# mkeeter/fidget

Hardware: AMD Instinct MI355X
Metric: Mvoxel/s (interval+point eval) on prospero.vm 1024^3 (higher is better)
Workload: dtype f32; 1 GPU; prospero.vm 3D heightmap+normals 1024^3, HipShape render hints (the library's tiles: 128/32/8, or 32/8 when the root level has few tiles), world_to_model=I

## Files before the change

fidget_amd/csrc/capi_core.hpp:

```cpp
struct DevBuf {
    void* p = nullptr;
    size_t cap = 0;
    hipError_t ensure(size_t bytes) {
        if (bytes <= cap) return hipSuccess;
        if (p) (void)hipFree(p);
        p = nullptr; cap = 0;
        hipError_t e = hipMalloc(&p, bytes);
        if (e == hipSuccess) cap = bytes;
        return e;
    }
    void release() { if (p) (void)hipFree(p); p = nullptr; cap = 0; }
};

static std::atomic<uint64_t> g_tape_serial{1};
struct BoundCache {
    struct Entry {
        uint64_t hash = 0, used = 0;
        std::vector<uint64_t> key;
        std::shared_ptr<const fhip_tape> tape;
    };
    std::mutex lock;
    std::vector<Entry> entries;
    uint64_t clock = 0;
};
// ... 52 lines not shown
#define X(name, dflt) {#name, &FhOptions::name},
    FH_OPTION_LIST(X)
#undef X
};
static void options_from_env(FhOptions& o) {
    for (const FhOptionEntry& e : FH_OPTION_TABLE) {
        std::string var = "FHIP_";
        for (const char* c = e.name; *c; c++) var += (char)toupper((unsigned char)*c);
        if (const char* v = getenv(var.c_str())) o.*(e.field) = *v ? atoi(v) : 1;
    }
}

struct FrameBufs {
    DevBuf state, arena, leaves, leaf_table, zbuf, normals, fp_lists, mind, squeue, slots[2], leaves_b, leaf_table_b, fp_lists_b, chw[2], tvals, topch, chwr, gscratch, rare_scratch;
    DevBuf queue[FH_MAX_LEVELS];
    uint32_t frame_stamp = 0;
    uint64_t resident_serial = 0;
    uint32_t resident_groups = 0;
    uint32_t forked = 0;
    bool async_pending = false;
    hipEvent_t ev_done = nullptr;
    bool ev_done_valid = false;
    std::shared_ptr<const fhip_tape> bound_hold;
    void release_all() {
        DevBuf* bufs[] = {&state, &arena, &leaves, &leaf_table, &zbuf, &normals, &fp_lists, &mind, &squeue, &slots[0], &slots[1],
                          &leaves_b, &leaf_table_b, &fp_lists_b, &chw[0], &chw[1], &tvals, &topch, &chwr, &gscratch, &rare_scratch};
        for (DevBuf* b : bufs) b->release();
        for (auto& q : queue) q.release();
        if (ev_done) (void)hipEventDestroy(ev_done);
        ev_done = nullptr;
        bound_hold.reset();
    }
};
struct fhip_ctx : FrameBufs {
    FhOptions opt;
#define FH_EXTRA_SETS 4
    FrameBufs others[FH_EXTRA_SETS];
    uint32_t extra_sets = 3;
    bool frame_pipeline = true;
    hipStream_t stream_pre = nullptr;
    uint32_t pre_turn = 0;
    hipEvent_t ev_rest_fork = nullptr, ev_rest_join = nullptr;
    hipEvent_t ev_pre = nullptr, ev_l0 = nullptr, ev_l1 = nullptr;
    hipModule_t asm_mod = nullptr;
    hipFunction_t asm_fn[FH_ASM_COUNT] = {};
    bool use_asm = true;
    bool probe = false;
// ... 204 lines not shown
```

fidget_amd/csrc/capi_render.hpp:

```cpp
static fhip_status bind_inputs(fhip_ctx* ctx, const fhip_tape* tape, const int32_t* axis_slots, const uint64_t* keys,
                               const float* vals, uint32_t n, FhRender& P) {
    const fh::HostTape& t = tape->t;
    std::vector<char> bound(FH_MAX_INPUTS, 0);
    for (uint32_t s = 0; s < FH_MAX_INPUTS; s++) { P.in_kind[s] = 3; P.in_value[s] = 0.0f; }
    for (int a = 0; a < 3; a++) {
        const int s = axis_slots ? axis_slots[a] : t.vars.axis[a];
        if (s >= 0 && s < FH_MAX_INPUTS) { P.in_kind[s] = (uint32_t)a; bound[s] = 1; }
    }
    for (uint32_t i = 0; i < n; i++) {
        const int s = axis_slots ? (int)keys[i] : t.vars.slot_of(3, keys[i]);
        if (s >= 0 && s < FH_MAX_INPUTS) { P.in_value[s] = vals[i]; bound[s] = 1; }
    }
    for (uint32_t s = 0; s < t.n_vars; s++)
        if (!bound[s]) return fail(ctx, FHIP_ERR_MISSING_VAR, "a variable of the shape has no value");
    return FHIP_OK;
}

struct HostSpans {
    double t[8] = {0, 0, 0, 0, 0, 0, 0, 0};
    uint64_t n = 0;
    std::chrono::steady_clock::time_point last;
    void start() { last = std::chrono::steady_clock::now(); }
    void mark(int k) { const auto now = std::chrono::steady_clock::now(); t[k] += std::chrono::duration<double, std::micro>(now - last).count(); last = now; }
    void frame() {
// ... 309 lines not shown
        kp.big = 1; kp.max_choices = R.S.P.max_choices;
        (void)launch_asm(ctx, fs.on(), FH_ASM_PRUNE1, bound, &kp, sizeof(kp));
    }
}
static void tiles_hip(fhip_ctx* ctx, const RenderSetup& R, FhRenderState* dS, int level, hipStream_t st) {
    const int gs = blocks_for(ctx, R.lds_tiles_small, 8), gb = blocks_big(ctx, R, R.lds_tiles_big, 8);
    if (level > 0 && R.full) FH_KLAUNCH((k_teval3d<true, false>), dim3(gs), dim3(WAVE), R.lds_tiles_small, st, dS, level);
    else if (level > 0) FH_KLAUNCH((k_teval3d<false, false>), dim3(gs), dim3(WAVE), R.lds_tiles_small, st, dS, level);
    if (R.full) FH_KLAUNCH((k_teval3d<true, true>), dim3(gb), dim3(WAVE), R.lds_tiles_big, st, dS, level);
    else FH_KLAUNCH((k_teval3d<false, true>), dim3(gb), dim3(WAVE), R.lds_tiles_big, st, dS, level);
}
static void launch_tiles_mono(fhip_ctx* ctx, const RenderSetup& R, FhRenderState* dS, int level, bool is3d, hipStream_t st) {
    const int gs = blocks_for(ctx, R.lds_tiles_small, 8), gb = blocks_big(ctx, R, R.lds_tiles_big, 8);
    launch(ctx, st, FHIP_K_TILES, [&] {
        if (is3d) { if (R.full) FH_LAUNCH_TILES(true, true, true, gb, R.lds_tiles_big); else FH_LAUNCH_TILES(true, false, true, gb, R.lds_tiles_big); }
        else { if (R.full) FH_LAUNCH_TILES(false, true, true, gb, R.lds_tiles_big); else FH_LAUNCH_TILES(false, false, true, gb, R.lds_tiles_big); }
    });
    if (level > 0)
        launch(ctx, st, FHIP_K_TILES, [&] {
            if (is3d) { if (R.full) FH_LAUNCH_TILES(true, true, false, gs, R.lds_tiles_small); else FH_LAUNCH_TILES(true, false, false, gs, R.lds_tiles_small); }
            else { if (R.full) FH_LAUNCH_TILES(false, true, false, gs, R.lds_tiles_small); else FH_LAUNCH_TILES(false, false, false, gs, R.lds_tiles_small); }
        });
}
static void launch_tiles(fhip_ctx* ctx, const RenderSetup& R, const LevelPlan& L, FhRenderState* dS, int level, bool is3d, FrameStreams& fs) {
    if (L.path == LevelPlan::MONO) return launch_tiles_mono(ctx, R, dS, level, is3d, fs.on());
    const int gp = ctx->n_cu * 8;
    launch(ctx, fs.on(), FHIP_K_TILES, [&] {
        if (is3d) FH_KLAUNCH(k_tsetup3d, dim3(gp), dim3(WAVE), 0, fs.on(), dS, level);
        else FH_KLAUNCH(k_tsetup2d, dim3(gp), dim3(WAVE), 0, fs.on(), dS, level);
    });
    launch(ctx, fs.on(), FHIP_K_TILES, [&] {
        if (L.path == LevelPlan::GROUPS) tiles_by_groups(ctx, R, dS, fs.on());
        else if (L.path == LevelPlan::ASM) tiles_asm(ctx, R, L, dS, level, fs);
        else tiles_hip(ctx, R, dS, level, fs.on());
    });
    const bool last = level + 1 == (int)R.S.P.n_levels;
    const int gpush = last ? ctx->n_cu * L.push_mul : gp;
    launch(ctx, fs.on(), FHIP_K_TILES, [&] {
        const uint32_t rb = L.rare ? FH_RARE_BLOCKS : 0u;
        if (is3d) FH_KLAUNCH(k_tpush3d, dim3(gpush + rb, last ? 1 : 17), dim3(WAVE), 0, fs.on(), dS, level, rb, rare_file(ctx, dS, L.rare_stride), L.rare_stride);
        else {
            if (!R.classify_only) FH_KLAUNCH(k_tpush2d, dim3(gpush), dim3(WAVE), 0, fs.on(), dS, level);
            const uint32_t slots_max = R.S.qcap[level] * ((level == 0 && R.groups) ? R.S.n_tgroups : 1u);
            FH_KLAUNCH(k_tfill2d, dim3(64, slots_max), dim3(256), 0, fs.on(), dS, level);
        }
    });
}

static fhip_status render2d_frame(fhip_ctx* ctx, const fhip_tape* tape, const fhip_render2d_config* cfg, float* out,
                                  int out_is_device) {
    if (ctx->is_cancelled()) return fail(ctx, FHIP_ERR_CANCELLED, "cancelled");
// ... 88 lines not shown
    HIP_TRY(ctx, hipEventRecord(ctx->ev_done, ctx->stream));
    ctx->ev_done_valid = true;
    if (!out_is_device) {
        HIP_TRY(ctx, hipMemcpyAsync(out, d_out, npix * 4, hipMemcpyDeviceToHost, ctx->stream));
        return finish_render(ctx);
    }
    return FHIP_OK;
}

static void slab_begin(fhip_ctx* ctx, const RenderSetup& R, const FrameSchedule& F, FhRenderState* dS, int k, hipStream_t st) {
    const FhRender& P = R.S.P;
    const uint32_t pre = R.S.pre_levels, n_groups = R.groups_per_slab, n32 = ((P.width + 31) / 32) * ((P.height + 31) / 32);
    launch(ctx, st, FHIP_K_OTHER, [&] {
        const bool pyr3 = P.n_levels == 3 && P.tiles[2] == 8 && P.tiles[1] == 32 && P.tiles[0] == 128 && n32 <= 1024;
        const bool rebuild = k != F.slab_first;
        const bool pyr2 = P.n_levels == 2 && P.tiles[1] == 8 && P.tiles[0] == 32 && pre == 1;
        if (rebuild && pyr2) { FH_KLAUNCH(k_slab_begin2, dim3(n32 + F.reset_blocks), dim3(256), 0, st, dS, n32, F.table_words, (uint32_t)k, n_groups); return; }
        if (rebuild && pyr3 && pre == 2) { FH_KLAUNCH(k_slab_begin3, dim3(n32 + F.reset_blocks), dim3(256), 0, st, dS, n32, F.table_words, (uint32_t)k, n_groups); return; }
        FH_KLAUNCH(k_reset_slab, dim3(F.reset_blocks * 4), dim3(WAVE), 0, st, dS, F.table_words, (uint32_t)k, n_groups, (pyr3 && rebuild) ? 1u : 0u);
        if (rebuild && pyr3) FH_KLAUNCH(k_minpyramid3, dim3(n32), dim3(256), 0, st, dS);
        else if (rebuild) FH_KLAUNCH(k_minpyramid, dim3(P.roots_x * P.roots_y), dim3(256), 0, st, dS);
    });
}
static fhip_status tile_step(fhip_ctx* ctx, const RenderSetup& R, const FrameSchedule& F, FrameStreams& fs, FhRenderState* dS, int k, int idx) {
    fs.cur = F.tiles;
    if (F.pipe && idx >= (int)F.NC) HIP_TRY(ctx, hipStreamWaitEvent(fs.on(), ctx->ev_leaves[idx - (int)F.NC], 0));
    slab_begin(ctx, R, F, dS, k, fs.on());
    for (uint32_t l = R.S.pre_levels; l < R.S.P.n_levels; l++) launch_tiles(ctx, R, F.level[l], dS, (int)l, true, fs);
    if (F.pipe) HIP_TRY(ctx, hipEventRecord(ctx->ev_tiles[idx], fs.on()));
    fs.cur = CALLER;
    return FHIP_OK;
}
static void classify_work(fhip_ctx* ctx, const RenderSetup& R, const FrameSchedule& F, FhRenderState* dS, hipStream_t st) {
    const uint32_t class_blocks = (R.n_footprints + FH_CLASSIFY_FP - 1) / FH_CLASSIFY_FP;
    if (F.by_list && F.rare && R.S.P.max_regs > R.S.leaf_asm_regs)
        launch(ctx, st, FHIP_K_OTHER, [&] { FH_KLAUNCH(k_classify3d, dim3(FH_RARE_BLOCKS), dim3(WAVE), 0, st, dS, 1, 0u, rare_file(ctx, dS, F.rare_stride), F.rare_stride); });
    else if (!F.by_list) launch(ctx, st, FHIP_K_OTHER, [&] {
        FH_KLAUNCH(k_classify3d, dim3(class_blocks + (F.rare ? FH_RARE_BLOCKS : 0u)), dim3(R.S.P.slab / 8 > 16 ? 256 : WAVE), 0, st, dS, R.asm_points ? 1 : 0, class_blocks,
                   rare_file(ctx, dS, F.rare_stride), F.rare_stride);
    });
    if (R.S.P.max_regs > R.S.leaf_asm_regs && !F.rare)
        launch(ctx, st, FHIP_K_POINTS, [&] {
            const int g = blocks_big(ctx, R, R.lds_points_big, 16);
            if (R.full) FH_KLAUNCH((k_leaves3d<2, 0, 1, true>), dim3(g), dim3(WAVE), R.lds_points_big, st, dS);
            else FH_KLAUNCH((k_leaves3d<2, 0, 1, false>), dim3(g), dim3(WAVE), R.lds_points_big, st, dS);
        });
}
static void leaf_work(fhip_ctx* ctx, const RenderSetup& R, const FrameSchedule& F, FhRenderState* dS, uint32_t sk, hipStream_t st) {
    launch(ctx, st, FHIP_K_POINTS, [&] {
        if (F.leaf_walk == FrameSchedule::HIP_LEAVES) {
            const int per_cu = R.full ? 8 : 16;
// ... 24 lines not shown
    launch(ctx, st, FHIP_K_NORMALS, [&] {
        const int gs = blocks_for(ctx, R.lds_normals_small, 8), gb = blocks_big(ctx, R, R.lds_normals_big, 8);
        const int which = R.asm_points_t ? FH_ASM_NORMALS_T : FH_ASM_NORMALS;
        if (F.by_list) {
            if (F.rare && R.S.P.max_regs > R.S.norm_asm_regs)
                FH_KLAUNCH(k_hits3d, dim3(FH_RARE_BLOCKS), dim3(WAVE), 0, st, dS, z_lo, z_hi, R.hit_bucket_cap, 0u, rare_file(ctx, dS, F.rare_stride), F.rare_stride);
            KaNormals kn = {dS, F.list_waves, R.col_slots, z_lo, z_hi, R.hit_bucket_cap, 1u};
            (void)launch_asm(ctx, st, which, kn.n_waves, &kn, sizeof(kn));
        }
        else if (R.asm_normals) {
            const uint32_t hb = std::min<uint32_t>(R.n_footprints, (uint32_t)ctx->n_cu * 64);
            FH_KLAUNCH(k_hits3d, dim3(hb + (F.rare ? FH_RARE_BLOCKS : 0u)), dim3(WAVE), 0, st, dS, z_lo, z_hi, R.hit_bucket_cap, hb, rare_file(ctx, dS, F.rare_stride), F.rare_stride);
            KaNormals kn = {dS, std::max<uint32_t>((uint32_t)(ctx->n_cu * 8) / FH_HIT_BUCKETS, 1u) * FH_HIT_BUCKETS, R.col_slots, z_lo, z_hi, R.hit_bucket_cap, 0};
            (void)launch_asm(ctx, st, which, kn.n_waves, &kn, sizeof(kn));
        }
        else if (R.full) FH_KLAUNCH((k_normals3d<true, false>), dim3(gs), dim3(WAVE), R.lds_normals_small, st, dS, z_lo, z_hi);
        else FH_KLAUNCH((k_normals3d<false, false>), dim3(gs), dim3(WAVE), R.lds_normals_small, st, dS, z_lo, z_hi);
        if (R.S.P.max_regs > R.S.norm_asm_regs && !(F.rare && R.asm_normals)) {
            if (R.full) FH_KLAUNCH((k_normals3d<true, true>), dim3(gb), dim3(WAVE), R.lds_normals_big, st, dS, z_lo, z_hi);
            else FH_KLAUNCH((k_normals3d<false, true>), dim3(gb), dim3(WAVE), R.lds_normals_big, st, dS, z_lo, z_hi);
        }
    });
}
static fhip_status coarse_levels(fhip_ctx* ctx, const RenderSetup& R, const FrameSchedule& F, FrameStreams& fs, FhRenderState* dS) {
    const uint32_t pre = R.S.pre_levels;
    FhFork fork{};
    fork.n = F.NC; fork.mark = F.coarse ? 1u : 0u;
    fork.leaves = (FhLeaf*)ctx->leaves_b.p; fork.leaf_table = (FhLeafRef*)ctx->leaf_table_b.p; fork.fp_lists = (uint32_t*)ctx->fp_lists_b.p;
    fork.leaf_cap = (size_t)R.S.leaf_cap; fork.n_footprints = (size_t)R.n_footprints; fork.hit_words = R.hit_words;
    const bool forked_here = F.coarse && R.zrep;
    if (F.coarse) {
        launch_tiles(ctx, R, F.level[0], dS, 0, true, fs);
        if (pre > 1) {
            HIP_TRY(ctx, hop(fs, F.l1_flags, ctx->ev_l0));
            if (R.zrep) launch(ctx, fs.on(), FHIP_K_OTHER, [&] { FH_KLAUNCH(k_tape_flags, dim3(ctx->n_cu * 4), dim3(WAVE), 0, fs.on(), dS, 1, R.col_depmask, 0, FhFork{}); });
            HIP_TRY(ctx, hop(fs, F.l1, ctx->ev_l0));
            launch_tiles(ctx, R, F.level[1], dS, 1, true, fs);
        }
        HIP_TRY(ctx, hop(fs, F.fork_on, pre > 1 ? ctx->ev_l1 : ctx->ev_l0));
        if (R.zrep) launch(ctx, fs.on(), FHIP_K_OTHER, [&] { FH_KLAUNCH(k_tape_flags, dim3(ctx->n_cu * 8 + 1), dim3(WAVE), 0, fs.on(), dS, (int)pre, R.col_depmask, 1, fork); });
        if (!F.pipe && !forked_here) launch(ctx, fs.on(), FHIP_K_OTHER, [&] { FH_KLAUNCH(k_mark_frame, dim3(1), dim3(1), 0, fs.on(), dS); });
    }
    if (F.pipe) {
        if (!forked_here) FH_KLAUNCH(k_fork_state, dim3(1), dim3(1), 0, fs.on(), dS, fork);
        HIP_TRY(ctx, hipEventRecord(ctx->ev_fork, fs.on()));
        if (F.fork_to_side) HIP_TRY(ctx, hipStreamWaitEvent(fs.s[SIDE], ctx->ev_fork, 0));
    }
    if (F.ev_pre) HIP_TRY(ctx, hop(fs, CALLER, ctx->ev_pre));
    fs.cur = CALLER;
    if (F.fork_to_tail) HIP_TRY(ctx, hipStreamWaitEvent(fs.s[TAIL], ctx->ev_fork, 0));
    return FHIP_OK;
}
static fhip_status render_slabs(fhip_ctx* ctx, const RenderSetup& R, const FrameSchedule& F, FrameStreams& fs, FhRenderState* dS0) {
    auto slab_state = [&](int idx) { return dS0 + (F.pipe ? (uint32_t)idx % F.NC : 0u); };
    for (int idx = 0; F.tiles_first && idx < F.n_rendered; idx++) { const fhip_status st = tile_step(ctx, R, F, fs, slab_state(idx), F.slab_first - idx, idx); if (st) return st; }
    for (int idx = 0; idx < F.n_rendered; idx++) {
        if (ctx->is_cancelled()) return fail(ctx, FHIP_ERR_CANCELLED, "cancelled");
        const int k = F.slab_first - idx;
        FhRenderState* const dS = slab_state(idx);
        if (!F.tiles_first) { const fhip_status st = tile_step(ctx, R, F, fs, dS, k, idx); if (st) return st; }
        if (F.pipe) HIP_TRY(ctx, hipStreamWaitEvent(fs.s[F.leaf], ctx->ev_tiles[idx], 0));
        if (F.aux_edge) HIP_TRY(ctx, hipStreamWaitEvent(fs.s[F.lists], ctx->ev_tiles[idx], 0));
        classify_work(ctx, R, F, dS, fs.s[F.lists]);
        leaf_work(ctx, R, F, dS, (uint32_t)(dS - dS0), fs.s[F.leaf]);
        if (F.aux_edge) { HIP_TRY(ctx, hipEventRecord(ctx->ev_aux[idx], fs.s[F.leaf])); HIP_TRY(ctx, hipStreamWaitEvent(fs.s[F.normals], ctx->ev_aux[idx], 0)); }
        if (F.normals_on) normals_work(ctx, R, F, dS, k, fs.s[F.normals]);
        if (F.pipe) HIP_TRY(ctx, hipEventRecord(ctx->ev_leaves[idx], fs.s[F.normals]));
    }
    if (F.aux_edge && F.n_rendered > 0) HIP_TRY(ctx, hipStreamWaitEvent(fs.s[CALLER], ctx->ev_leaves[F.n_rendered - 1], 0));
    return FHIP_OK;
}

static fhip_status render3d_frame(fhip_ctx* ctx, const fhip_tape* tape, const fhip_render3d_config* cfg, void* out,
                                  int out_is_device, const PartSpec& part) {
    if (ctx->is_cancelled()) return fail(ctx, FHIP_ERR_CANCELLED, "cancelled");
    if (ctx->opt.stats & 2) g_spans.start();
    (void)hipSetDevice(ctx->device);
    RenderSetup R;
    memset(&R.S, 0, sizeof(R.S));
    FhRender& P = R.S.P;
    P.width = cfg->width; P.height = cfg->height; P.depth = cfg->depth; P.z = 0; P.pixel_perfect = 0;
    fhip_status st = bind_inputs(ctx, tape, cfg->axis_slots, cfg->var_keys, cfg->var_values, cfg->n_vars, P);
    if (st) return st;
    const uint32_t size[3] = {cfg->width, cfg->height, cfg->depth};
    float s2w[16];
    const float ident[16] = {1, 0, 0, 0, 0, 1, 0, 0, 0, 0, 1, 0, 0, 0, 0, 1};
    fhip_screen_to_world(size, 3, s2w);
    mat_product(cfg->world_to_model ? cfg->world_to_model : ident, s2w, 4, P.mat);
    const TapeFacts facts = tape_facts(tape);
    const PlanInputs pin = plan_inputs(ctx);
    column_facts(P, facts, pin, R);
    const TileChoice tiles = choose_tiles_3d(cfg->tile_sizes, cfg->n_tile_sizes, size, part.n_shards * part.nx * part.ny, part.nz, R.column_inv, pin.root32_max, pin.no_zrep,
                                             linked_root_tape(facts, pin));
    if (!tiles.valid) return fail(ctx, FHIP_ERR_UNSUPPORTED, "bad tile size list");
    if (tiles.substituted) ctx->substituted_tiles++;
    ScheduleInputs in = schedule_inputs(ctx, out_is_device);
    in.huge = (size_t)std::max<uint32_t>(tape->t.n_regs, 1) * WAVE * 16 > FH_LDS_MAX || tiles_lds(std::max<uint32_t>(tape->t.n_regs, 1), tape->t.n_choices, 64) > FH_LDS_MAX;
    in.whole = part.n_shards == 1 && part.nx * part.ny * part.nz == 1;
    if (frame_pipelined(in)) {
        for (uint32_t i = 0; i < ctx->extra_sets; i++) std::swap(static_cast<FrameBufs&>(*ctx), ctx->others[i]);
        in.frames_queued = ctx->extra_sets > 0 && ctx->others[0].ev_done_valid && hipEventQuery(ctx->others[0].ev_done) == hipErrorNotReady;
        (void)hipGetLastError();
    }
    FH_SPAN(0);
    st = prepare(ctx, tape, facts, true, tiles.ts, part, R);
    if (st) return st;
    FH_SPAN(1);
    in.pre_turn = ctx->pre_turn;
    if (ctx->host_flags) { in.rare_seen = ctx->host_flags[2]; in.last_leaves = ctx->host_flags[3]; }
    const FrameSchedule F = schedule_frame(R, in);
    if (F.takes_turn) ctx->pre_turn++;
    if (F.rare) { HIP_TRY(ctx, ctx->rare_scratch.ensure((size_t)F.rare_stride * FH_RARE_BLOCKS * 4)); ctx->rare_frames++; }
    R.S.leaf_list = F.by_list ? 1u : 0u; ctx->forked = F.pipe ? F.NC : 0;
    FrameStreams fs = frame_streams(ctx, F.root);
    if (F.fpipe && ctx->ev_done_valid) HIP_TRY(ctx, hipStreamWaitEvent(fs.on(), ctx->ev_done, 0));
    const size_t npix = (size_t)cfg->width * cfg->height;
    FhGeometryPixel* d_out = (FhGeometryPixel*)out;
    if (!out_is_device) { HIP_TRY(ctx, ctx->tmp_out.ensure(npix * sizeof(FhGeometryPixel))); d_out = (FhGeometryPixel*)ctx->tmp_out.p; }
    FhRenderState* const dS0 = (FhRenderState*)ctx->state.p;
    const FrameClear clear3[3] = {{ctx->zbuf.p, npix * 8, 0u}, {ctx->normals.p, npix * 12, 0u}, {ctx->mind.p, R.mind_words * 4, 0u}};
    st = upload_frame(ctx, fs.on(), tape, R, clear3);
    if (st) return st;
    FH_SPAN(2);
    st = coarse_levels(ctx, R, F, fs, dS0);
    if (st) return st;
    FH_SPAN(3);
    st = render_slabs(ctx, R, F, fs, dS0);
    if (st) return st;
    FH_SPAN(4);
    launch(ctx, ctx->stream, FHIP_K_OTHER, [&] { FH_KLAUNCH(k_finish3d, dim3(ctx->n_cu * 16), dim3(WAVE), 0, ctx->stream, dS0, d_out, std::max<uint32_t>(ctx->forked, 1u), (uint32_t*)ctx->sticky.p, ctx->host_flags); });
    HIP_TRY(ctx, hipGetLastError());
    if (ctx->launch_failed) { ctx->launch_failed = false; return FHIP_ERR_HIP; }
    ctx->async_pending = out_is_device != 0;
    HIP_TRY(ctx, hipEventRecord(ctx->ev_done, ctx->stream));
    ctx->ev_done_valid = true;
    if (ctx->opt.stats & 2) { g_spans.mark(5); g_spans.frame(); }
    if (!out_is_device) {
        HIP_TRY(ctx, hipMemcpyAsync(out, d_out, npix * sizeof(FhGeometryPixel), hipMemcpyDeviceToHost, ctx->stream));
        return finish_render(ctx);
    }
    return FHIP_OK;
}
static bool lanes_possible(fhip_ctx* ctx, int out_is_device) {
    if (ctx->opt.frame_lanes < 2 || ctx->is_lane || !out_is_device || ctx->profiling || ctx->probe || (ctx->opt.stats & 1)) return false;
    if (!ctx->ev_last_valid) return false;
    const hipError_t q = hipEventQuery(ctx->ev_last);
    (void)hipGetLastError();
    return q == hipErrorNotReady;
}
static void lane_tune_release(fhip_ctx* ctx);
static void lanes_release(fhip_ctx* ctx, bool keep_measurements) {
    if (!keep_measurements) lane_tune_release(ctx);
    for (fhip_ctx* L : ctx->lanes) {
        hipStream_t const s = L->lane_stream_owned ? L->stream : nullptr;
        if (L->lane_done) (void)hipEventDestroy(L->lane_done);
        if (L->lane_copied) (void)hipEventDestroy(L->lane_copied);
        L->lane_img.release();
        fhip_ctx_destroy(L);
// ... 211 lines not shown
```

fidget_amd/csrc/frame_plan.hpp:

```cpp
#pragma once
#include <stddef.h>
#include <stdint.h>
#include <string.h>

#include <algorithm>
#include <vector>

#include "render_state.h"

static const uint32_t VM_TILES_2D[] = {128, 32, 8};
static const uint32_t VM_TILES_3D[] = {128, 64, 32, 16, 8};
static const uint32_t FH_LEAF_REGS = 40, FH_LEAF_REGS_T = 44;
static const uint32_t FH_NORMAL_REGS = 40;
static const uint32_t HIP_TILES_2D[] = {128, 16};
static const uint32_t MID_REGS = 64, MID_CHOICES = 768;
static size_t tiles_lds(uint32_t regs, uint32_t choices, uint32_t TL) {
    size_t b = (size_t)regs * TL * 8 + (size_t)((choices + 15) / 16) * TL * 4 + (size_t)regs * TL + 256;
    return (b + 15) & ~(size_t)15;
}

struct PartSpec {
    uint32_t shard = 0, n_shards = 1;
    uint32_t ix = 0, nx = 1, iy = 0, ny = 1, iz = 0, nz = 1;
};
// ... 324 lines not shown
        const size_t words[2] = {(SMALL_CHOICES + 15) / 16, ((size_t)P.max_choices + 15) / 16};
        for (int k = 0; k < 2; k++) B.chw[k] = std::max<size_t>(cap * words[k] * 256, 256);
    }
    if (R.split) {
        uint32_t cap = 1;
        for (size_t l = 0; l < ts.size(); l++) cap = std::max(cap, qcaps[l] * (l == 0 && R.groups ? S.n_tgroups : 1u));
        B.slots = (size_t)cap * sizeof(FhSlot);
        S.slot_cap[0] = S.slot_cap[1] = cap;
    }
    S.arena_frame_end = S.arena_root_end;
    R.zrep = R.split && S.pre_levels > 0 && R.xy_fixed && !in.no_column_inv && in.no_zrep != 1;
    if (((size_t)t.n_ops + 64) * 8 > in.arena_bytes) return refuse(PLAN_UNSUPPORTED, "tape larger than the arena");
    std::reverse(R.roots.begin(), R.roots.end());
    return PlanStatus{};
}

static void plan_linked_prune(const TapeFacts& t, const PlanInputs& in, bool has_links, uint32_t n_chain, RenderSetup& R) {
    R.p2_cap_kept = (uint32_t)FH_P2_MAX_KEPT;
    R.lds_prune2 = (size_t)FH_P2_WPB * fh_p2_wave_lds(t.n_choices, R.p2_cap_kept) + (((size_t)n_chain * 4 + 15) & ~(size_t)15);
    R.n_chain = n_chain;
    R.prune2 = R.groups && has_links && linked_root_tape(t, in) && R.lds_prune2 <= FH_LDS_MAX &&
               R.roots.size() * 64 <= (size_t)2 * in.n_cu * FH_P2_WPB;
}
```

fidget_amd/csrc/kernels.hip:

```cpp
#include <hip/hip_runtime.h>

#include "dev_ops.hpp"
#include "render_state.h"

using namespace fhd;

#define AS4 __attribute__((address_space(4)))
typedef const AS4 uint64_t* ctape_t;

typedef unsigned long long Q4 __attribute__((ext_vector_type(4), aligned(8)));
FH_DEV uint64_t q4_pick(Q4 q, int u) { return u == 0 ? q.x : (u == 1 ? q.y : (u == 2 ? q.z : q.w)); }

FH_DEV uint32_t uni(uint32_t v) { return __builtin_amdgcn_readfirstlane(v); }
FH_DEV uint32_t arena_reserve(FhRenderState* S, uint32_t n) {
    const uint32_t base = atomicAdd(&S->arena_head, n);
    if (base + n < base || base + n > S->arena_cap) { atomicMin(&S->arena_head, S->arena_cap); return 0xFFFFFFFFu; }
    return base;
}
FH_DEV uint64_t ballot(bool p) { return __ballot(p); }

FH_DEV bool op_is_heavy(uint32_t op) {
    return (op >= FH_SIN && op <= FH_LN) || op == FH_ATAN2_RR || op == FH_ATAN2_RI || op == FH_ATAN2_IR ||
           op == FH_MOD_RR || op == FH_MOD_RI || op == FH_MOD_IR;
}
// ... 439 lines not shown

struct FhFork {
    uint32_t n, mark;
    FhLeaf* leaves; FhLeafRef* leaf_table; uint32_t* fp_lists;
    size_t leaf_cap, n_footprints, hit_words;
};
FH_DEV void fork_state_body(FhRenderState* A, const FhFork& f) {
    if (f.mark) A->arena_frame_end = min(A->arena_head, A->arena_cap);
    const uint32_t n = f.n;
    const uint32_t lo = min(A->pre_levels ? A->arena_frame_end : A->arena_root_end, A->arena_cap);
    const uint32_t part = (A->arena_cap - lo) / n;
    for (uint32_t k = 1; k < n; k++) {
        FhRenderState* B = A + k;
        *B = *A;
        B->leaves = f.leaves + (k - 1) * f.leaf_cap; B->leaf_table = f.leaf_table + (k - 1) * f.leaf_cap;
        uint32_t* fp = f.fp_lists + (k - 1) * (3 * f.n_footprints + f.hit_words);
        B->fp_list[0] = fp; B->fp_list[1] = fp + f.n_footprints; B->fp_list[2] = fp + 2 * f.n_footprints; B->hit_list = fp + 3 * f.n_footprints;
        B->arena_frame_end = lo + k * part; B->arena_root_end = lo + k * part;
        B->arena_cap = lo + (k + 1) * part;
    }
    A->arena_cap = lo + part;
}
__global__ void k_fork_state(FhRenderState* A, FhFork f) { fork_state_body(A, f); }

__global__ void __launch_bounds__(WAVE) k_tape_flags(FhRenderState* S, int level, uint32_t depmask, int parked, FhFork fork) {
    const uint32_t n_blocks = gridDim.x - (fork.n ? 1u : 0u);
    if (blockIdx.x >= n_blocks) {
        if (threadIdx.x == 0) fork_state_body(S, fork);
        return;
    }
    const int lane = threadIdx.x;
    const uint32_t nq = parked ? S->n_slabs : 1u;
    for (uint32_t q = 0; q < nq; q++) {
        FhGroup* const base = parked ? S->squeue + (size_t)q * S->squeue_cap : S->queue[level];
        const uint32_t cap = parked ? S->squeue_cap : S->qcap[level];
        const uint32_t ns = parked ? S->scount[q] : S->count[level], nb = parked ? S->scount_big[q] : S->count_big[level];
        for (uint32_t gi = blockIdx.x; gi < ns + nb; gi += n_blocks) {
            FhGroup& g = base[gi < ns ? gi : cap - 1 - (gi - ns)];
            const ctape_t tape = (ctape_t)(S->arena + g.tape.off);
            const uint32_t len = uni(g.tape.len);
            bool dep = false;
            for (uint32_t k = lane; k < len; k += WAVE) {
                const uint64_t w = tape[k];
                if ((uint32_t)(w & 0xFFu) == FH_INPUT && ((depmask >> ((uint32_t)(w >> 32) & 31u)) & 1u)) dep = true;
            }
            const bool any = ballot(dep) != 0;
            if (lane == 0) g.stride = any ? 0u : 0x80000000u;
        }
    }
}

template <bool IS3D>
FH_DEV void tsetup_body(FhRenderState* S, int level) {
    const AS4 FhRender& P = *(const AS4 FhRender*)&S->P;
    const int lane = threadIdx.x;
    const uint32_t T = P.tiles[level];
    const uint32_t ntx = (P.width + T - 1) / T;
    const uint32_t* mind = S->mind[level];
    Mat4 mat;
#pragma unroll
    for (int i = 0; i < 16; i++) mat.m[i] = P.mat[i];
    const uint32_t TG = (level == 0 && S->n_tgroups) ? S->n_tgroups : 1;
    const uint32_t G = TG;
    const uint32_t ns = min(S->count[level], S->slot_cap[0] / G), nb = min(S->count_big[level], S->slot_cap[1] / G);
    if (blockIdx.x == 0 && lane == 0) {
        S->n_slots[0][level] = ns * G; S->n_slots[1][level] = nb * G;
        if (IS3D && nb && S->pre_levels > 0 && (uint32_t)level >= S->pre_levels) S->rare_seen = 1u;
    }
    const uint32_t parts = TG > 1 ? max(1u, min(TG, gridDim.x / max(ns + nb, 1u))) : 1u;
    for (uint32_t wi = blockIdx.x; wi < (ns + nb) * parts; wi += gridDim.x) {
        const uint32_t gi = wi / parts, part = wi % parts;
        const bool big = gi >= ns;
        const AS4 FhGroup& g = *(const AS4 FhGroup*)&S->queue[level][big ? S->qcap[level] - 1 - (gi - ns) : gi];
        FhSlot* const slg = &S->slots[big ? 1 : 0][(big ? (gi - ns) : gi) * G];
        FhSlot& sl = *slg;
        const uint32_t zrep = (IS3D && level > 0 && g.n > 1) ? g.n : 1u;
        const bool inv = IS3D && level > 0 && ((g.stride >> 31) != 0 || zrep > 1);
        if (IS3D && level > 0) {
            const uint32_t Tp = P.tiles[level - 1], ntxp = (P.width + Tp - 1) / Tp;
            if (S->mind[level - 1][(g.y / Tp) * ntxp + g.x / Tp] >= g.z + (zrep - 1) * Tp + Tp + 1) { if (lane < (int)G && part == 0) slg[lane].act = 0; continue; }
        }
        uint32_t nchild, cx, cy, cz;
        const uint32_t copies0 = (IS3D && level == 0 && g.x > 1) ? g.x : 1u;
        if (level == 0) {
            nchild = g.n;
            const uint32_t ri = g.first + lane * g.stride;
            cx = (ri / P.roots_y) * T; cy = (ri % P.roots_y) * T; cz = g.z;
        } else {
            const uint32_t n = P.tiles[level - 1] / T;
            nchild = IS3D ? n * n * n : n * n;
            cx = g.x + (lane % n) * T; cy = g.y + ((lane / n) % n) * T; cz = IS3D ? g.z + (lane / (n * n)) * T : 0u;
        }
        bool act = lane < (int)nchild && cx < P.width && cy < P.height;
        uint32_t cz_top = cz + (copies0 - 1) * T;
        if (inv) {
            const uint32_t n = P.tiles[level - 1] / T;
            if (lane / (n * n) != 0) act = false;
            cz_top = g.z + (zrep - 1) * P.tiles[level - 1] + (n - 1) * T;
        }
        if (IS3D && act && mind[(cy / T) * ntx + cx / T] >= cz_top + T + 1) act = false;
        const uint64_t actm = ballot(act);
        if (actm == 0) { if (lane < (int)G && part == 0) slg[lane].act = 0; continue; }
        IV X, Y, Z;
        xf_interval(mat, iv((float)cx, (float)cx + (float)T), iv((float)cy, (float)cy + (float)T),
                    IS3D ? iv((float)cz, (float)cz + (float)T) : iv(P.z, P.z), X, Y, Z);
        for (uint32_t k = part; k < G; k += parts) {
            FhSlot& so = slg[k];
            const uint64_t share = actm;
            if (lane == 0) {
                const FhTapeRef tr = (TG > 1) ? S->tgroup[k] : FhTapeRef{g.tape.off, g.tape.len, g.tape.n_regs, g.tape.n_choices};
                so.tape = tr;
                so.level = (uint32_t)level | (copies0 << 8); so.act = share; so.base = 0; so.overflow = 0;
                so.tvals = (TG > 1) ? S->tvals + (size_t)(gi - ns) * S->n_terms * WAVE * 2 : (float*)(uintptr_t)((inv ? 1u : 0u) | (zrep << 8));
            }
            if (share == 0) continue;
            so.xyz[0][lane] = X.lo; so.xyz[1][lane] = X.hi; so.xyz[2][lane] = Y.lo; so.xyz[3][lane] = Y.hi;
            so.xyz[4][lane] = Z.lo; so.xyz[5][lane] = Z.hi;
            so.corner[0][lane] = cx; so.corner[1][lane] = cy; so.corner[2][lane] = cz;
        }
    }
}

__global__ void __launch_bounds__(WAVE) k_tsetup3d(FhRenderState* S, int level) { tsetup_body<true>(S, level); }
__global__ void __launch_bounds__(WAVE) k_tsetup2d(FhRenderState* S, int level) { tsetup_body<false>(S, level); }

FH_DEV IV top_comb(bool is_min, IV a, IV b) {
    if (iv_has_nan(a) || iv_has_nan(b)) return iv_nan();
    return is_min ? iv(rmin(a.lo, b.lo), rmin(a.hi, b.hi)) : iv(rmax(a.lo, b.lo), rmax(a.hi, b.hi));
}
#define FH_CHAIN_SEG 16
__global__ void __launch_bounds__(WAVE) k_tchain3d(FhRenderState* S) {
    const int lane = threadIdx.x;
    const uint32_t c = blockIdx.x, b = blockIdx.y, G = S->n_tgroups, n_top = S->n_top;
    if (b >= S->n_slots[1][0] / G) return;
    FhSlot& p = S->slots[1][(size_t)b * G];
    if (((p.act >> c) & 1) == 0) return;
    const IV* const tv = (const IV*)S->tvals + (size_t)b * S->n_terms * WAVE;
    uint8_t* const tc = S->topch + ((size_t)b * WAVE + c) * n_top;
    const uint32_t* const top = (const uint32_t*)S->ttop;
    const bool is_min = (top[0] & 0xFF) == FH_MIN_RR || (top[0] & 0xFF) == FH_MIN_RI;
    const float ident = is_min ? u2f(0x7f800000u) : u2f(0xff800000u);
    const uint32_t per = (n_top + WAVE - 1) / WAVE, j0 = (uint32_t)lane * per;
    IV e[FH_CHAIN_SEG];
#pragma unroll
    for (int k = 0; k < FH_CHAIN_SEG; k++) {
        const uint32_t j = j0 + k;
// ... 859 lines not shown
        const uint32_t tx = bx * 4 + i, x = tx * T1 + (lane & 7);
        uint32_t mn = (x < P.width && y < P.height) ? (uint32_t)(S->zbuf[(size_t)y * P.width + x] >> 32) : 0xFFFFFFFFu;
#pragma unroll
        for (int d = 32; d >= 1; d >>= 1) mn = min(mn, (uint32_t)__shfl_xor((int)mn, d, WAVE));
        if (lane == 0 && tx * T1 < P.width && ty * T1 < P.height) S->mind[1][ty * n1x + tx] = mn;
        row = min(row, mn);
    }
    if (lane == 0) part[w] = row;
    __syncthreads();
    if (threadIdx.x == 0) S->mind[0][by * n0x + bx] = min(min(part[0], part[1]), min(part[2], part[3]));
}
__global__ void __launch_bounds__(256) k_slab_begin2(FhRenderState* S, uint32_t n0, uint32_t table_words, uint32_t slab, uint32_t n_root_groups) {
    if (blockIdx.x < n0) { minpyramid2_body(S, blockIdx.x); return; }
    reset_slab_body(S, (blockIdx.x - n0) * blockDim.x + threadIdx.x, (gridDim.x - n0) * blockDim.x, table_words, slab, n_root_groups, 0);
}

FH_DEV void latch_arena(const FhRenderState* S, uint32_t n_ctx, volatile uint32_t* host_flags) {
    uint32_t a = 0, peak = 0;
    for (uint32_t k = 0; k < n_ctx; k++) { a |= S[k].arena_overflow; peak = max(peak, S[k].arena_head); }
    if (a) host_flags[0] = 1u;
    if (peak > host_flags[1]) host_flags[1] = peak;
}
__global__ void k_latch_arena(const FhRenderState* S, uint32_t n_ctx, volatile uint32_t* host_flags) { latch_arena(S, n_ctx, host_flags); }
__global__ void k_finish3d(FhRenderState* S, FhGeometryPixel* out, uint32_t n_ctx, uint32_t* sticky, volatile uint32_t* host_flags) {
    const AS4 FhRender& P = *(const AS4 FhRender*)&S->P;
    const size_t n = (size_t)P.width * P.height;
    if (blockIdx.x == 0 && threadIdx.x == 0 && sticky) {
        uint32_t q = 0;
        for (uint32_t k = 0; k < n_ctx; k++) q |= S[k].queue_overflow;
        if (q) atomicOr(sticky, 1u);
        if (host_flags) {
            latch_arena(S, n_ctx, host_flags);
            uint32_t r = 0;
            for (uint32_t k = 0; k < n_ctx; k++) r |= S[k].rare_seen;
            host_flags[2] = r;
            uint32_t nl = 0;
            for (uint32_t k = 0; k < n_ctx; k++) nl = max(nl, S[k].n_leaves);
            host_flags[3] = nl;
        }
    }
    for (size_t i = blockIdx.x * (size_t)blockDim.x + threadIdx.x; i < n; i += (size_t)gridDim.x * blockDim.x) {
        const uint32_t d = (uint32_t)(S->zbuf[i] >> 32);
        FhGeometryPixel o;
        if (d >= P.depth - 1) { o.normal[0] = 0.0f; o.normal[1] = 0.0f; o.normal[2] = 1.0f; o.depth = P.depth; }
        else { o.normal[0] = S->normals[i * 3]; o.normal[1] = S->normals[i * 3 + 1]; o.normal[2] = S->normals[i * 3 + 2]; o.depth = d; }
        out[i] = o;
    }
}

__global__ void k_merge_depth(FhGeometryPixel* front, const FhGeometryPixel* back, size_t n, uint32_t D) {
    for (size_t i = (size_t)blockIdx.x * blockDim.x + threadIdx.x; i < n; i += (size_t)gridDim.x * blockDim.x) {
        FhGeometryPixel a = front[i];
        const FhGeometryPixel b = back[i];
        if (b.depth > a.depth) a = b;
        if (D && a.depth >= D - 1) { a.depth = D; a.normal[0] = 0.0f; a.normal[1] = 0.0f; a.normal[2] = 1.0f; }
        front[i] = a;
    }
}

__global__ void k_math_sweep(int op, uint32_t first, uint32_t stride, size_t n, const float* __restrict__ ref, unsigned long long* out) {
    unsigned long long worst = 0, ndiff = 0, nbad = 0;
    for (size_t i = (size_t)blockIdx.x * blockDim.x + threadIdx.x; i < n; i += (size_t)gridDim.x * blockDim.x) {
        const uint32_t xb = first + (uint32_t)i * stride;
        const float x = u2f(xb);
        float y;
        switch (op) {
            case 0: y = t_sin(x); break;
            case 1: y = t_cos(x); break;
            case 2: y = t_tan(x); break;
// ... 64 lines not shown
```

Measured before the change: 9.733 million Mvoxel/s.

## Clear frame buffers in finish kernel and fold tape flags into tile setup

```diff
diff --git a/fidget_amd/csrc/capi_core.hpp b/fidget_amd/csrc/capi_core.hpp
--- a/fidget_amd/csrc/capi_core.hpp
+++ b/fidget_amd/csrc/capi_core.hpp
@@ -98,7 +98,9 @@
     hipEvent_t ev_done = nullptr;
     bool ev_done_valid = false;
     std::shared_ptr<const fhip_tape> bound_hold;
+    CleanSig clean;
     void release_all() {
+        clean = CleanSig();
         DevBuf* bufs[] = {&state, &arena, &leaves, &leaf_table, &zbuf, &normals, &fp_lists, &mind, &squeue, &slots[0], &slots[1],
                           &leaves_b, &leaf_table_b, &fp_lists_b, &chw[0], &chw[1], &tvals, &topch, &chwr, &gscratch, &rare_scratch};
         for (DevBuf* b : bufs) b->release();
diff --git a/fidget_amd/csrc/capi_render.hpp b/fidget_amd/csrc/capi_render.hpp
--- a/fidget_amd/csrc/capi_render.hpp
+++ b/fidget_amd/csrc/capi_render.hpp
@@ -355,11 +355,11 @@
             else { if (R.full) FH_LAUNCH_TILES(false, true, false, gs, R.lds_tiles_small); else FH_LAUNCH_TILES(false, false, false, gs, R.lds_tiles_small); }
         });
 }
-static void launch_tiles(fhip_ctx* ctx, const RenderSetup& R, const LevelPlan& L, FhRenderState* dS, int level, bool is3d, FrameStreams& fs) {
+static void launch_tiles(fhip_ctx* ctx, const RenderSetup& R, const LevelPlan& L, FhRenderState* dS, int level, bool is3d, FrameStreams& fs, const FhHead* head = nullptr) {
     if (L.path == LevelPlan::MONO) return launch_tiles_mono(ctx, R, dS, level, is3d, fs.on());
     const int gp = ctx->n_cu * 8;
     launch(ctx, fs.on(), FHIP_K_TILES, [&] {
-        if (is3d) FH_KLAUNCH(k_tsetup3d, dim3(gp), dim3(WAVE), 0, fs.on(), dS, level);
+        if (is3d) FH_KLAUNCH(k_tsetup3d, dim3(gp), dim3(WAVE), 0, fs.on(), dS, level, head ? *head : FhHead{});
         else FH_KLAUNCH(k_tsetup2d, dim3(gp), dim3(WAVE), 0, fs.on(), dS, level);
     });
     launch(ctx, fs.on(), FHIP_K_TILES, [&] {
@@ -494,11 +494,12 @@
         else if (rebuild) FH_KLAUNCH(k_minpyramid, dim3(P.roots_x * P.roots_y), dim3(256), 0, st, dS);
     });
 }
-static fhip_status tile_step(fhip_ctx* ctx, const RenderSetup& R, const FrameSchedule& F, FrameStreams& fs, FhRenderState* dS, int k, int idx) {
+static fhip_status tile_step(fhip_ctx* ctx, const RenderSetup& R, const FrameSchedule& F, FrameStreams& fs, FhRenderState* dS, int k, int idx, const FhHead* head) {
     fs.cur = F.tiles;
     if (F.pipe && idx >= (int)F.NC) HIP_TRY(ctx, hipStreamWaitEvent(fs.on(), ctx->ev_leaves[idx - (int)F.NC], 0));
-    slab_begin(ctx, R, F, dS, k, fs.on());
-    for (uint32_t l = R.S.pre_levels; l < R.S.P.n_levels; l++) launch_tiles(ctx, R, F.level[l], dS, (int)l, true, fs);
+    const FhHead* const mine = head && idx == 0 ? head : nullptr;
+    if (!mine) slab_begin(ctx, R, F, dS, k, fs.on());
+    for (uint32_t l = R.S.pre_levels; l < R.S.P.n_levels; l++) launch_tiles(ctx, R, F.level[l], dS, (int)l, true, fs, l == R.S.pre_levels ? mine : nullptr);
     if (F.pipe) HIP_TRY(ctx, hipEventRecord(ctx->ev_tiles[idx], fs.on()));
     fs.cur = CALLER;
     return FHIP_OK;
@@ -569,12 +570,19 @@
         }
     });
 }
-static fhip_status coarse_levels(fhip_ctx* ctx, const RenderSetup& R, const FrameSchedule& F, FrameStreams& fs, FhRenderState* dS) {
-    const uint32_t pre = R.S.pre_levels;
-    FhFork fork{};
+static FhHead tile_head(const fhip_ctx* ctx, const RenderSetup& R, const FrameSchedule& F) {
+    FhHead h{};
+    FhFork& fork = h.fork;
     fork.n = F.NC; fork.mark = F.coarse ? 1u : 0u;
     fork.leaves = (FhLeaf*)ctx->leaves_b.p; fork.leaf_table = (FhLeafRef*)ctx->leaf_table_b.p; fork.fp_lists = (uint32_t*)ctx->fp_lists_b.p;
     fork.leaf_cap = (size_t)R.S.leaf_cap; fork.n_footprints = (size_t)R.n_footprints; fork.hit_words = R.hit_words;
+    h.on = F.coarse && R.zrep && R.S.pre_levels == 1 && F.by_list && F.n_rendered > 0 && F.level[1].path != LevelPlan::MONO ? 1u : 0u;
+    h.slab = (uint32_t)F.slab_first; h.n_root_groups = R.groups_per_slab; h.depmask = R.col_depmask;
+    return h;
+}
+static fhip_status coarse_levels(fhip_ctx* ctx, const RenderSetup& R, const FrameSchedule& F, FrameStreams& fs, FhRenderState* dS, const FhHead& head) {
+    const uint32_t pre = R.S.pre_levels;
+    const FhFork& fork = head.fork;
     const bool forked_here = F.coarse && R.zrep;
     if (F.coarse) {
         launch_tiles(ctx, R, F.level[0], dS, 0, true, fs);
@@ -585,7 +593,7 @@
             launch_tiles(ctx, R, F.level[1], dS, 1, true, fs);
         }
         HIP_TRY(ctx, hop(fs, F.fork_on, pre > 1 ? ctx->ev_l1 : ctx->ev_l0));
-        if (R.zrep) launch(ctx, fs.on(), FHIP_K_OTHER, [&] { FH_KLAUNCH(k_tape_flags, dim3(ctx->n_cu * 8 + 1), dim3(WAVE), 0, fs.on(), dS, (int)pre, R.col_depmask, 1, fork); });
+        if (R.zrep && !head.on) launch(ctx, fs.on(), FHIP_K_OTHER, [&] { FH_KLAUNCH(k_tape_flags, dim3(ctx->n_cu * 8 + 1), dim3(WAVE), 0, fs.on(), dS, (int)pre, R.col_depmask, 1, fork); });
         if (!F.pipe && !forked_here) launch(ctx, fs.on(), FHIP_K_OTHER, [&] { FH_KLAUNCH(k_mark_frame, dim3(1), dim3(1), 0, fs.on(), dS); });
     }
     if (F.pipe) {
@@ -598,14 +606,18 @@
     if (F.fork_to_tail) HIP_TRY(ctx, hipStreamWaitEvent(fs.s[TAIL], ctx->ev_fork, 0));
     return FHIP_OK;
 }
-static fhip_status render_slabs(fhip_ctx* ctx, const RenderSetup& R, const FrameSchedule& F, FrameStreams& fs, FhRenderState* dS0) {
+static fhip_status render_slabs(fhip_ctx* ctx, const RenderSetup& R, const FrameSchedule& F, FrameStreams& fs, FhRenderState* dS0, const FhHead& head) {
+    const FhHead* const hd = head.on ? &head : nullptr;
     auto slab_state = [&](int idx) { return dS0 + (F.pipe ? (uint32_t)idx % F.NC : 0u); };
-    for (int idx = 0; F.tiles_first && idx < F.n_rendered; idx++) { const fhip_status st = tile_step(ctx, R, F, fs, slab_state(idx), F.slab_first - idx, idx); if (st) return st; }
+    for (int idx = 0; F.tiles_first && idx < F.n_rendered; idx++) { const fhip_status st = tile_step(ctx, R, F, fs, slab_state(idx), F.slab_first - idx, idx, hd); if (st) return st; }
     for (int idx = 0; idx < F.n_rendered; idx++) {
-        if (ctx->is_cancelled()) return fail(ctx, FHIP_ERR_CANCELLED, "cancelled");
+        if (ctx->is_cancelled()) {
+            if (hd && idx == 0 && !F.tiles_first) ctx->forked = 0;
+            return fail(ctx, FHIP_ERR_CANCELLED, "cancelled");
+        }
         const int k = F.slab_first - idx;
         FhRenderState* const dS = slab_state(idx);
-        if (!F.tiles_first) { const fhip_status st = tile_step(ctx, R, F, fs, dS, k, idx); if (st) return st; }
+        if (!F.tiles_first) { const fhip_status st = tile_step(ctx, R, F, fs, dS, k, idx, hd); if (st) return st; }
         if (F.pipe) HIP_TRY(ctx, hipStreamWaitEvent(fs.s[F.leaf], ctx->ev_tiles[idx], 0));
         if (F.aux_edge) HIP_TRY(ctx, hipStreamWaitEvent(fs.s[F.lists], ctx->ev_tiles[idx], 0));
         classify_work(ctx, R, F, dS, fs.s[F.lists]);
@@ -649,6 +661,8 @@
         in.frames_queued = ctx->extra_sets > 0 && ctx->others[0].ev_done_valid && hipEventQuery(ctx->others[0].ev_done) == hipErrorNotReady;
         (void)hipGetLastError();
     }
+    const CleanSig left_clean = ctx->clean;
+    ctx->clean = CleanSig();
     FH_SPAN(0);
     st = prepare(ctx, tape, facts, true, tiles.ts, part, R);
     if (st) return st;
@@ -665,22 +679,29 @@
     FhGeometryPixel* d_out = (FhGeometryPixel*)out;
     if (!out_is_device) { HIP_TRY(ctx, ctx->tmp_out.ensure(npix * sizeof(FhGeometryPixel))); d_out = (FhGeometryPixel*)ctx->tmp_out.p; }
     FhRenderState* const dS0 = (FhRenderState*)ctx->state.p;
-    const FrameClear clear3[3] = {{ctx->zbuf.p, npix * 8, 0u}, {ctx->normals.p, npix * 12, 0u}, {ctx->mind.p, R.mind_words * 4, 0u}};
-    st = upload_frame(ctx, fs.on(), tape, R, clear3);
+    const CleanFrame kind = {out_is_device != 0, ctx->profiling};
+    CleanSig want_clean;
+    want_clean.valid = true; want_clean.pixels = npix; want_clean.mind_words = R.mind_words;
+    const bool is_clean = set_is_clean(left_clean, want_clean);
+    const FrameClear clear3[3] = {{ctx->zbuf.p, npix * 8, 0u}, {ctx->normals.p, npix * 12, 0u}, {ctx->mind.p, R.mind_words * 4, 0u}}, no_clear[3] = {};
+    st = upload_frame(ctx, fs.on(), tape, R, is_clean ? no_clear : clear3);
     if (st) return st;
     FH_SPAN(2);
-    st = coarse_levels(ctx, R, F, fs, dS0);
+    const FhHead head = tile_head(ctx, R, F);
+    st = coarse_levels(ctx, R, F, fs, dS0, head);
     if (st) return st;
     FH_SPAN(3);
-    st = render_slabs(ctx, R, F, fs, dS0);
+    st = render_slabs(ctx, R, F, fs, dS0, head);
     if (st) return st;
     FH_SPAN(4);
-    launch(ctx, ctx->stream, FHIP_K_OTHER, [&] { FH_KLAUNCH(k_finish3d, dim3(ctx->n_cu * 16), dim3(WAVE), 0, ctx->stream, dS0, d_out, std::max<uint32_t>(ctx->forked, 1u), (uint32_t*)ctx->sticky.p, ctx->host_flags); });
+    launch(ctx, ctx->stream, FHIP_K_OTHER, [&] { FH_KLAUNCH(k_finish3d, dim3(ctx->n_cu * 16), dim3(WAVE), 0, ctx->stream, dS0, d_out, std::max<uint32_t>(ctx->forked, 1u), (uint32_t*)ctx->sticky.p, ctx->host_flags,
+                                                            leaves_set_clean(kind) ? 1u : 0u, (uint32_t)R.mind_words); });
     HIP_TRY(ctx, hipGetLastError());
     if (ctx->launch_failed) { ctx->launch_failed = false; return FHIP_ERR_HIP; }
     ctx->async_pending = out_is_device != 0;
     HIP_TRY(ctx, hipEventRecord(ctx->ev_done, ctx->stream));
     ctx->ev_done_valid = true;
+    ctx->clean = set_left_by(kind, want_clean, true);
     if (ctx->opt.stats & 2) { g_spans.mark(5); g_spans.frame(); }
     if (!out_is_device) {
         HIP_TRY(ctx, hipMemcpyAsync(out, d_out, npix * sizeof(FhGeometryPixel), hipMemcpyDeviceToHost, ctx->stream));
diff --git a/fidget_amd/csrc/frame_plan.hpp b/fidget_amd/csrc/frame_plan.hpp
--- a/fidget_amd/csrc/frame_plan.hpp
+++ b/fidget_amd/csrc/frame_plan.hpp
@@ -370,3 +370,20 @@
     R.prune2 = R.groups && has_links && linked_root_tape(t, in) && R.lds_prune2 <= FH_LDS_MAX &&
                R.roots.size() * 64 <= (size_t)2 * in.n_cu * FH_P2_WPB;
 }
+
+struct CleanSig {
+    bool valid = false;
+    uint64_t pixels = 0, mind_words = 0;
+};
+struct CleanFrame {
+    bool out_is_device = true, profiling = false;
+};
+static bool leaves_set_clean(const CleanFrame& f) { return f.out_is_device && !f.profiling; }
+static bool set_is_clean(const CleanSig& left, const CleanSig& want) {
+    return left.valid && want.valid && left.pixels == want.pixels && left.mind_words == want.mind_words;
+}
+static CleanSig set_left_by(const CleanFrame& f, const CleanSig& want, bool queued_whole) {
+    CleanSig s = want;
+    s.valid = want.valid && queued_whole && leaves_set_clean(f);
+    return s;
+}
diff --git a/fidget_amd/csrc/kernels.hip b/fidget_amd/csrc/kernels.hip
--- a/fidget_amd/csrc/kernels.hip
+++ b/fidget_amd/csrc/kernels.hip
@@ -485,6 +485,20 @@
     A->arena_cap = lo + part;
 }
 __global__ void k_fork_state(FhRenderState* A, FhFork f) { fork_state_body(A, f); }
+FH_DEV uint32_t tape_flag(const FhRenderState* S, uint32_t off, uint32_t len, uint32_t depmask, int lane) {
+    const ctape_t tape = (ctape_t)(S->arena + off);
+    bool dep = false;
+    for (uint32_t k = lane; k < len; k += WAVE) {
+        const uint64_t w = tape[k];
+        if ((uint32_t)(w & 0xFFu) == FH_INPUT && ((depmask >> ((uint32_t)(w >> 32) & 31u)) & 1u)) dep = true;
+    }
+    return ballot(dep) != 0 ? 0u : 0x80000000u;
+}
+struct FhHead {
+    uint32_t on, slab, n_root_groups, depmask;
+    FhFork fork;
+};
+FH_DEV void reset_slab_body(FhRenderState* S, uint32_t i, uint32_t stride, uint32_t table_words, uint32_t slab, uint32_t n_root_groups, uint32_t reset_root_mind);
 
 __global__ void __launch_bounds__(WAVE) k_tape_flags(FhRenderState* S, int level, uint32_t depmask, int parked, FhFork fork) {
     const uint32_t n_blocks = gridDim.x - (fork.n ? 1u : 0u);
@@ -500,21 +514,14 @@
         const uint32_t ns = parked ? S->scount[q] : S->count[level], nb = parked ? S->scount_big[q] : S->count_big[level];
         for (uint32_t gi = blockIdx.x; gi < ns + nb; gi += n_blocks) {
             FhGroup& g = base[gi < ns ? gi : cap - 1 - (gi - ns)];
-            const ctape_t tape = (ctape_t)(S->arena + g.tape.off);
-            const uint32_t len = uni(g.tape.len);
-            bool dep = false;
-            for (uint32_t k = lane; k < len; k += WAVE) {
-                const uint64_t w = tape[k];
-                if ((uint32_t)(w & 0xFFu) == FH_INPUT && ((depmask >> ((uint32_t)(w >> 32) & 31u)) & 1u)) dep = true;
-            }
-            const bool any = ballot(dep) != 0;
-            if (lane == 0) g.stride = any ? 0u : 0x80000000u;
+            const uint32_t flag = tape_flag(S, uni(g.tape.off), uni(g.tape.len), depmask, lane);
+            if (lane == 0) g.stride = flag;
         }
     }
 }
 
 template <bool IS3D>
-FH_DEV void tsetup_body(FhRenderState* S, int level) {
+FH_DEV void tsetup_body(FhRenderState* S, int level, const FhHead* head = nullptr) {
     const AS4 FhRender& P = *(const AS4 FhRender*)&S->P;
     const int lane = threadIdx.x;
     const uint32_t T = P.tiles[level];
@@ -525,7 +532,14 @@
     for (int i = 0; i < 16; i++) mat.m[i] = P.mat[i];
     const uint32_t TG = (level == 0 && S->n_tgroups) ? S->n_tgroups : 1;
     const uint32_t G = TG;
-    const uint32_t ns = min(S->count[level], S->slot_cap[0] / G), nb = min(S->count_big[level], S->slot_cap[1] / G);
+    const bool hd = IS3D && head && head->on;
+    const FhGroup* const queue = hd ? S->squeue + (size_t)head->slab * S->squeue_cap : S->queue[level];
+    const uint32_t cnt = hd ? S->scount[head->slab] : S->count[level], cnt_big = hd ? S->scount_big[head->slab] : S->count_big[level];
+    if (hd && blockIdx.x == 0) {
+        if (lane == 0 && head->fork.n) fork_state_body(S, head->fork);
+        reset_slab_body(S, (uint32_t)lane, WAVE, 0u, head->slab, head->n_root_groups, 0u);
+    }
+    const uint32_t ns = min(cnt, S->slot_cap[0] / G), nb = min(cnt_big, S->slot_cap[1] / G);
     if (blockIdx.x == 0 && lane == 0) {
         S->n_slots[0][level] = ns * G; S->n_slots[1][level] = nb * G;
         if (IS3D && nb && S->pre_levels > 0 && (uint32_t)level >= S->pre_levels) S->rare_seen = 1u;
@@ -534,15 +548,15 @@
     for (uint32_t wi = blockIdx.x; wi < (ns + nb) * parts; wi += gridDim.x) {
         const uint32_t gi = wi / parts, part = wi % parts;
         const bool big = gi >= ns;
-        const AS4 FhGroup& g = *(const AS4 FhGroup*)&S->queue[level][big ? S->qcap[level] - 1 - (gi - ns) : gi];
+        const AS4 FhGroup& g = *(const AS4 FhGroup*)&queue[big ? S->qcap[level] - 1 - (gi - ns) : gi];
         FhSlot* const slg = &S->slots[big ? 1 : 0][(big ? (gi - ns) : gi) * G];
         FhSlot& sl = *slg;
         const uint32_t zrep = (IS3D && level > 0 && g.n > 1) ? g.n : 1u;
-        const bool inv = IS3D && level > 0 && ((g.stride >> 31) != 0 || zrep > 1);
         if (IS3D && level > 0) {
             const uint32_t Tp = P.tiles[level - 1], ntxp = (P.width + Tp - 1) / Tp;
             if (S->mind[level - 1][(g.y / Tp) * ntxp + g.x / Tp] >= g.z + (zrep - 1) * Tp + Tp + 1) { if (lane < (int)G && part == 0) slg[lane].act = 0; continue; }
         }
+        const bool inv = IS3D && level > 0 && (zrep > 1 || ((hd ? tape_flag(S, g.tape.off, g.tape.len, head->depmask, lane) : g.stride) >> 31) != 0);
         uint32_t nchild, cx, cy, cz;
         const uint32_t copies0 = (IS3D && level == 0 && g.x > 1) ? g.x : 1u;
         if (level == 0) {
@@ -584,7 +598,7 @@
     }
 }
 
-__global__ void __launch_bounds__(WAVE) k_tsetup3d(FhRenderState* S, int level) { tsetup_body<true>(S, level); }
+__global__ void __launch_bounds__(WAVE) k_tsetup3d(FhRenderState* S, int level, FhHead head) { tsetup_body<true>(S, level, &head); }
 __global__ void __launch_bounds__(WAVE) k_tsetup2d(FhRenderState* S, int level) { tsetup_body<false>(S, level); }
 
 FH_DEV IV top_comb(bool is_min, IV a, IV b) {
@@ -1490,9 +1504,11 @@
     if (peak > host_flags[1]) host_flags[1] = peak;
 }
 __global__ void k_latch_arena(const FhRenderState* S, uint32_t n_ctx, volatile uint32_t* host_flags) { latch_arena(S, n_ctx, host_flags); }
-__global__ void k_finish3d(FhRenderState* S, FhGeometryPixel* out, uint32_t n_ctx, uint32_t* sticky, volatile uint32_t* host_flags) {
+__global__ void k_finish3d(FhRenderState* S, FhGeometryPixel* out, uint32_t n_ctx, uint32_t* sticky, volatile uint32_t* host_flags, uint32_t leave_clean, uint32_t mind_words) {
     const AS4 FhRender& P = *(const AS4 FhRender*)&S->P;
     const size_t n = (size_t)P.width * P.height;
+    if (leave_clean)
+        for (size_t i = blockIdx.x * (size_t)blockDim.x + threadIdx.x; i < mind_words; i += (size_t)gridDim.x * blockDim.x) S->mind[0][i] = 0u;
     if (blockIdx.x == 0 && threadIdx.x == 0 && sticky) {
         uint32_t q = 0;
         for (uint32_t k = 0; k < n_ctx; k++) q |= S[k].queue_overflow;
@@ -1508,11 +1524,13 @@
         }
     }
     for (size_t i = blockIdx.x * (size_t)blockDim.x + threadIdx.x; i < n; i += (size_t)gridDim.x * blockDim.x) {
-        const uint32_t d = (uint32_t)(S->zbuf[i] >> 32);
+        const uint64_t zb = S->zbuf[i];
+        const uint32_t d = (uint32_t)(zb >> 32);
         FhGeometryPixel o;
         if (d >= P.depth - 1) { o.normal[0] = 0.0f; o.normal[1] = 0.0f; o.normal[2] = 1.0f; o.depth = P.depth; }
         else { o.normal[0] = S->normals[i * 3]; o.normal[1] = S->normals[i * 3 + 1]; o.normal[2] = S->normals[i * 3 + 2]; o.depth = d; }
         out[i] = o;
+        if (leave_clean && zb) { S->zbuf[i] = 0; S->normals[i * 3] = 0.0f; S->normals[i * 3 + 1] = 0.0f; S->normals[i * 3 + 2] = 0.0f; }
     }
 }
 
```

Measured after the change: 10.05 million Mvoxel/s (median of 6 runs). +3.2%, better.
